# shuwang127/SRCNN_Cpp

Measured on AMD Instinct MI355X. Metric: SRCNN Y-channel Mpixels/sec, higher is better.
Workload: dtype f32; 1 GPU; 1 x 3840x2160 luma plane per GPU per step (1920x1080 x2.0, BASELINE configs[1]), fused conv path, mfma arithmetic, inputs resident in HBM; frames_per_gpu=1, width=3840, height=2160, mode=mfma, seam_deferral=True, output_checksum=584152

## Files before the change

### srcnn_cpp_amd/csrc/srcnn_kernels.h

```cpp
#pragma once
#include <hip/hip_runtime.h>
#include <stddef.h>
#include <stdint.h>

namespace srcnn {

constexpr int FW = 128;
constexpr int YP = FW + 8;
constexpr int YR = 16;
constexpr int NWAVES = FW / 32;
constexpr int NTHREADS = NWAVES * 64;

enum StripMode { MODE_FUSED = 0, MODE_L12 = 1, MODE_L3 = 2 };

constexpr int NFRAG_L1 = 82;
constexpr int NFRAG_L2 = 32;
constexpr int NFRAG_L3 = 16;
constexpr int NFRAG_B2 = 16;
constexpr int NFRAG_L2U = 32;
constexpr int NFRAG_B2U = 16;
constexpr int NFRAG_L3U = 16;
constexpr int FRAG_L2 = NFRAG_L1, FRAG_L3 = FRAG_L2 + NFRAG_L2, FRAG_B2 = FRAG_L3 + NFRAG_L3,
              FRAG_L2U = FRAG_B2 + NFRAG_B2, FRAG_B2U = FRAG_L2U + NFRAG_L2U, FRAG_L3U = FRAG_B2U + NFRAG_B2U;
constexpr int NFRAG = FRAG_L3U + NFRAG_L3U;

__host__ __device__ constexpr int acc_row(int r, int h) { return (r & 3) + 8 * (r >> 2) + 4 * h; }
__host__ __device__ constexpr int row_chan(int i) { return 2 * ((i & 3) + 4 * (i >> 3)) + ((i >> 2) & 1); }

__host__ __device__ constexpr int l3_row_tap(int i)
{
    const int r = (i & 3) + 4 * (i >> 3), h = (i >> 2) & 1, s = r / 5, m = r % 5, n = h ? 3 + s : s;
    return (r < 15 && n < 5) ? 5 * m + n : -1;
}
__host__ __device__ constexpr bool l3_row_is_scale(int i)
{
    const int r = (i & 3) + 4 * (i >> 3), h = (i >> 2) & 1;
    return h == 1 && r >= 10 && r < 15;
}

constexpr int S16_FRAG_L2 = 24, S16_FRAG_L3 = 32, S16_NFRAG = 36;
constexpr size_t S16_TABLE_BYTES = (size_t)S16_NFRAG * 64 * 16 + 2 * 16 * sizeof(float);
__host__ __device__ constexpr int l1s_tap(int b, int h, int e)
{
    const int n = 4 * b + e / 2, u = e & 1;
    if (n < 20) return (2 * (n % 5) + u < 9) ? 9 * (n / 5 + 5 * h) + 2 * (n % 5) + u : -1;
    if (n < 23) {
        const int jj = 4 * h + 2 * (n - 20) + u;
        return (h == 0 ? jj <= 3 : (jj >= 4 && jj <= 8)) ? 36 + jj : -1;
    }
    return (u == 0 && h == 0) ? 81 : -1;
}

struct StripParams {
    const uint8_t *src;
    long src_stride, src_frame_pitch;
    int src_row0;
    const uint8_t *src_top, *src_bot;
    long halo_stride;
    int src_row1;
    const float *planes_in;
    float *planes_out;
    long pl_stride, pl_pitch, pl_frame_pitch;
    uint8_t *dst;
    float *pre;
    long dst_stride, dst_frame_pitch;
    int dst_row0;
    const float *wfrag;
    const uint32_t *wfrag16;
    float *sink;
    float b3;
    int width, height;
    int row_begin, row_end;
    int seg_rows, n_strips, n_segs;
    const int *items;
    int items_per_frame;
    int seams_per_frame;
    float *seam;
    float *cseam;
    int strips_total;
    int tune;
    uint8_t *flag;
    float fix_delta, fix_scale;
    float fix_kl, fix_abs;
    unsigned *fix_counters;
};

enum { FIX_N_SCAT = 0, FIX_N_DENSE = 1, FIX_N_CHANGED = 2, FIX_MAX_DEV = 3, FIX_N_RERUN = 4,
       FIX_MAX_RATIO = 5,
       FIX_TOTALS = 6,
       FIX_WORD_STRIDE = 64,
       FIX_NEXT_ITEM = 6,
       FIX_NEXT_RERUN = 7,
       FIX_REGIONS = 8, FIX_REGION0 = 8 * FIX_WORD_STRIDE,
       FIX_COUNTERS = FIX_REGION0 + FIX_REGIONS * FIX_WORD_STRIDE };
struct FixParams {
    const uint8_t *src;
    long src_stride;
    int src_row0;
    const uint8_t *src_top, *src_bot;
    long halo_stride;
    int src_row1;
    uint8_t *dst;
    const uint8_t *flag;
    long dst_stride;
    int dst_row0;
    int width, height, row_begin, row_end;
    const float *wraw;
// ... 172 lines not shown
```

### srcnn_cpp_amd/csrc/srcnn_mfma.hip

```cpp
#include "srcnn_kernels.h"

#include <type_traits>

#ifndef SRCNN_SAFE_HAZARDS
#define SRCNN_SAFE_HAZARDS 0
#endif
#if SRCNN_SAFE_HAZARDS
#define SRCNN_KNS safe
#else
#define SRCNN_KNS fast
#endif

namespace srcnn {
namespace SRCNN_KNS {

typedef float f32x16 __attribute__((ext_vector_type(16)));
typedef float f32x2 __attribute__((ext_vector_type(2)));

#define MFMA(a, b, c) __builtin_amdgcn_mfma_f32_32x32x2f32((a), (b), (c), 0, 0, 0)

__device__ __forceinline__ f32x16 mfma_first(float a, float b, const f32x16 &c)
{
#if SRCNN_SAFE_HAZARDS
    return MFMA(a, b, c);
#endif
    f32x16 d;
    asm volatile("v_mfma_f32_32x32x2_f32 %0, %1, %2, %3" : "=&v"(d) : "v"(a), "v"(b), "v"(c));
    return d;
}
__device__ __forceinline__ f32x16 mfma_first0(float a, float b)
{
#if SRCNN_SAFE_HAZARDS
    const f32x16 z = {0};
    return MFMA(a, b, z);
#endif
    f32x16 d;
    asm volatile("v_mfma_f32_32x32x2_f32 %0, %1, %2, 0" : "=&v"(d) : "v"(a), "v"(b));
    return d;
}


__device__ __forceinline__ int clampi(int v, int lo, int hi) { return min(max(v, lo), hi); }

__device__ __forceinline__ unsigned lane_off(unsigned x)
{
    asm volatile("" : "+v"(x));
    return x;
}
template <typename T>
__device__ __forceinline__ __attribute__((address_space(1))) T *scalar_base(T *p)
{
    __attribute__((address_space(1))) T *g = (__attribute__((address_space(1))) T *)p;
    asm volatile("" : "+s"(g));
    return g;
}

template <typename T>
__device__ __forceinline__ T *uniform_ptr(T *p)
{
    const unsigned long long a = (unsigned long long)p;
    const unsigned lo = __builtin_amdgcn_readfirstlane((unsigned)a), hi = __builtin_amdgcn_readfirstlane((unsigned)(a >> 32));
    return (T *)(((unsigned long long)hi << 32) | lo);
}

__device__ __forceinline__ void lds_barrier()
{
    asm volatile("s_waitcnt lgkmcnt(0)\n\ts_barrier" ::: "memory");
}

__device__ __forceinline__ float relu(float x)
{
    float r;
    asm("v_max_f32 %0, 0, %1" : "=v"(r) : "v"(x));
    return r;
}

__device__ const signed char CSEAM_TERMS[15][9] = {
    {4, 0, 124, 1, 125, 2, 126, 3, 127}, {3, 0, 125, 1, 126, 2, 127, 0, 0}, {1, 0, 126, 0, 0, 0, 0, 0, 0},
    {1, 0, 127, 0, 0, 0, 0, 0, 0},       {1, 1, 127, 0, 0, 0, 0, 0, 0},     {1, 2, 0, 0, 0, 0, 0, 0, 0},
    {1, 3, 1, 0, 0, 0, 0, 0, 0},         {1, 4, 2, 0, 0, 0, 0, 0, 0},       {1, 1, 0, 0, 0, 0, 0, 0, 0},
    {1, 2, 1, 0, 0, 0, 0, 0, 0},         {1, 3, 2, 0, 0, 0, 0, 0, 0},       {1, 4, 3, 0, 0, 0, 0, 0, 0},
    {1, 3, 0, 0, 0, 0, 0, 0, 0},         {1, 4, 0, 0, 0, 0, 0, 0, 0},       {1, 4, 1, 0, 0, 0, 0, 0, 0}};

struct CseamLane {
    int cnt, off[4];
};
__device__ __forceinline__ CseamLane cseam_lane(int e)
{
    CseamLane cl = {0, {0, 0, 0, 0}};
    if (e < 15) {
        const signed char *t = CSEAM_TERMS[e];
        cl.cnt = t[0];
#pragma unroll
        for (int i = 0; i < 4; ++i) cl.off[i] = i < t[0] ? t[1 + 2 * i] * FW + t[2 + 2 * i] : 0;
    }
    return cl;
}
__device__ __forceinline__ void cseam_export(const float *tile, float *dst, int e, const CseamLane &cl)
{
    const float a = tile[cl.off[0]], b = tile[cl.off[1]], c = tile[cl.off[2]], d = tile[cl.off[3]];
    float v = a;
    v = cl.cnt > 1 ? v + b : v;
    v = cl.cnt > 2 ? v + c : v;
    v = cl.cnt > 3 ? v + d : v;
    if (cl.cnt > 0) dst[(unsigned)e] = v;
}

__device__ __forceinline__ void relu_pairs(f32x16 &a, const f32x2 ones)
{
#if SRCNN_SAFE_HAZARDS
#pragma unroll
    for (int q = 0; q < 16; ++q) a[q] = __builtin_fmaxf(a[q], 0.f);
    return;
#endif
#pragma unroll
    for (int q = 0; q < 8; ++q) {
        f32x2 pr = {a[2 * q], a[2 * q + 1]};
        asm("v_pk_mul_f32 %0, %0, %1 clamp" : "+v"(pr) : "s"(ones));
        a[2 * q] = pr.x;
        a[2 * q + 1] = pr.y;
    }
}

constexpr bool fast_kernel(int mode, bool pre, int diag)
{
    (void)diag;
    return mode == MODE_FUSED && !pre;
}

template <int MODE, bool PRE, int DIAG = 0, bool FIX = false, bool HALO3 = false>
__device__ __forceinline__ void strip_body(const StripParams &p)
{
    static_assert(!FIX || (MODE == MODE_FUSED && !PRE && DIAG == 0), "flags belong to the production fused kernel");
    static_assert(!HALO3 || (MODE == MODE_FUSED && !PRE && DIAG == 0), "halo buffers belong to the production fused kernel");
    if constexpr (FIX) {
        if (blockIdx.x == 0)
            for (int i = threadIdx.x; i < FIX_COUNTERS; i += 256) p.fix_counters[i] = 0u;
    }
    unsigned long long lt[4] = {0, 0, 0, 0};
    if constexpr (DIAG == 2) lt[0] = __builtin_amdgcn_s_memrealtime();
    extern __shared__ __attribute__((aligned(16))) char smem[];
    float *ylds = reinterpret_cast<float *>(smem);
    float *fbuf = (MODE == MODE_L3) ? ylds : ylds + 2 * YR * YP;

    const int tid = threadIdx.x;
    const int lane = tid & 63;
    const int wave = __builtin_amdgcn_readfirstlane(tid >> 6);
    const int j = lane & 31;
    const int half = lane >> 5;

    constexpr int HALO = (MODE == MODE_L12) ? 0 : 2;

    const int W = p.width, H = p.height;
    int bid = blockIdx.x;
    int strip, frame = 0, ys, ye, seam_up = -1, seam_dn = -1;
    if (p.items) {
        frame = bid / p.items_per_frame;
        const int *it = p.items + ITEM_INTS * (bid - frame * p.items_per_frame);
        strip = it[0];
        ys = it[1];
        ye = it[2];
        if constexpr (MODE == MODE_FUSED) {
            seam_up = it[3] >= 0 ? it[3] + frame * p.seams_per_frame : -1;
            seam_dn = it[4] >= 0 ? it[4] + frame * p.seams_per_frame : -1;
        }
        if (ys >= ye) return;
    } else {
        if (!(p.tune & 8)) {
            const int nwg = gridDim.x, q = nwg >> 3, r = nwg & 7, xcd = bid & 7;
            bid = (xcd < r ? xcd * (q + 1) : r * (q + 1) + (xcd - r) * q) + (bid >> 3);
        }
        strip = bid % p.n_strips;
        bid /= p.n_strips;
        const int seg = bid % p.n_segs;
        frame = bid / p.n_segs;
        ys = p.row_begin + seg * p.seg_rows;
        ye = min(ys + p.seg_rows, p.row_end);
    }

    const bool cs = (MODE != MODE_L12) && p.cseam != nullptr;
    const CseamLane cl = cseam_lane((cs && threadIdx.x < 64 && (threadIdx.x & 31) < 15 &&
                                     (threadIdx.x < 32 || fast_kernel(MODE, PRE, DIAG)))
                                        ? (int)(threadIdx.x & 31) : 15);
    const int halo_c = cs ? 0 : HALO;
    const int xs = strip * (FW - 2 * halo_c);
    const int gx0 = xs - halo_c;
    float *cs_row0 = (cs && wave == 0)
                         ? p.cseam + (((long)frame * p.strips_total + strip) * (p.row_end - p.row_begin) - p.row_begin) * CSEAM_FLOATS
                         : nullptr;
    const bool top_open = seam_up >= 0, bot_open = seam_dn >= 0;
    const int f_lo = top_open ? ys : max(ys - HALO, 0);
    const int f_hi = bot_open ? ye : min(ye + HALO, H);
    const int out_lo = top_open ? ys + 2 : ys, out_hi = bot_open ? ye - 2 : ye;

    const float *wf = p.wfrag + lane;
    float w1f[2][41], w2f[32], w3f[16];
    f32x16 b2v = {0};
    if constexpr (MODE != MODE_L3) {
#pragma unroll
        for (int t = 0; t < 2; ++t)
#pragma unroll
            for (int s = 0; s < 41; ++s) w1f[t][s] = wf[(t * 41 + s) * 64];
        constexpr int L2 = (MODE == MODE_L12) ? FRAG_L2U : FRAG_L2, B2 = (MODE == MODE_L12) ? FRAG_B2U : FRAG_B2;
#pragma unroll
        for (int q = 0; q < 32; ++q) w2f[q] = wf[(L2 + q) * 64];
#pragma unroll
        for (int q = 0; q < 16; ++q) b2v[q] = wf[(B2 + q) * 64];
    }
    if constexpr (MODE != MODE_L12) {
        constexpr int L3 = (MODE == MODE_L3) ? FRAG_L3U : FRAG_L3;
#pragma unroll
        for (int q = 0; q < 16; ++q) w3f[q] = wf[(L3 + q) * 64];
    }
    const f32x2 ones = {1.0f, 1.0f};

    const uint8_t *srcf = nullptr;
    int ycol = 0;
    if constexpr (MODE != MODE_L3) {
        srcf = p.src + (long)frame * p.src_frame_pitch;
        ycol = clampi(gx0 - 4 + tid, 0, W - 1);
    }
    const int y_last = min(H - 1, f_hi + 3);
    auto y_row = [&](int r) -> const uint8_t * {
        if constexpr (HALO3) {
            if (r < p.src_row0) return p.src_top + (long)(r - (p.src_row0 - 6)) * p.halo_stride;
            if (r >= p.src_row1) return p.src_bot + (long)(r - p.src_row1) * p.halo_stride;
        }
        return srcf + (long)(r - p.src_row0) * p.src_stride;
    };
    auto load_y = [&](int r) -> uint8_t {
        const uint8_t *row = y_row(clampi(r, 0, y_last));
        return row[(unsigned)ycol];
    };
    auto stage_y = [&](int r, uint8_t v) {
        const int slot = r & (YR - 1);
        const float fv = (float)v;
        ylds[slot * YP + tid] = fv;
        ylds[(slot + YR) * YP + tid] = fv;
    };
    if constexpr (MODE != MODE_L3) {
        if (tid < YP) {
            uint8_t v[9];
#pragma unroll
            for (int q = 0; q < 9; ++q) v[q] = load_y(f_lo - 4 + q);
#pragma unroll
            for (int q = 0; q < 9; ++q) stage_y(f_lo - 4 + q, v[q]);
        }
        __syncthreads();
    }
    asm volatile("s_waitcnt vmcnt(0)" ::: "memory");
    if constexpr (MODE != MODE_L3) {
#pragma unroll
        for (int t = 0; t < 2; ++t)
#pragma unroll
            for (int k = 0; k < 41; ++k) asm volatile("" : "+v"(w1f[t][k]));
#pragma unroll
        for (int q = 0; q < 32; ++q) asm volatile("" : "+v"(w2f[q]));
        asm volatile("" : "+v"(b2v));
    }
    if constexpr (MODE != MODE_L12) {
#pragma unroll
        for (int q = 0; q < 16; ++q) asm volatile("" : "+v"(w3f[q]));
    }

    if constexpr (DIAG == 2) lt[1] = __builtin_amdgcn_s_memrealtime();

    const int xi = 32 * wave + j;
    const int gx = gx0 + xi;


    constexpr bool FASTK = fast_kernel(MODE, PRE, DIAG);
    static_assert(!FIX || FASTK, "the flag threshold reads plane 5 through the FAST kernels' column offsets");
    constexpr int FSLOT = 6 * FW;
    int xn[5] = {0, 0, 0, 0, 0};
    bool px_ok = false;
    if constexpr (MODE != MODE_L12) {
#pragma unroll
        for (int n = 0; n < 5; ++n) {
            xn[n] = clampi(clampi(gx + n - 2, 0, W - 1) - gx0, 0, FW - 1);
            if constexpr (FASTK) xn[n] += n * FW + half * FSLOT;
        }
        px_ok = cs ? (gx < W) && (xi >= 2 || strip == 0) && (xi < FW - 2 || strip == p.strips_total - 1)
                   : (xi >= HALO) && (xi < FW - HALO) && (gx < W);
    }
    CseamLane cl2 = cl;
    if constexpr (FASTK) {
#pragma unroll
        for (int i = 0; i < 4; ++i) cl2.off[i] += half * FSLOT;
    }
    float R[4][3] = {{0.f, 0.f, 0.f}, {0.f, 0.f, 0.f}, {0.f, 0.f, 0.f}, {0.f, 0.f, 0.f}};
    long o_out = (long)frame * p.dst_frame_pitch + (long)(f_lo - 3 - p.dst_row0) * p.dst_stride;
    long o_src = (long)(min(f_lo + 5, y_last) - p.src_row0) * p.src_stride;
    long o_pl = (long)frame * p.pl_frame_pitch + (long)(MODE == MODE_L3 ? min(f_lo + 1, H - 1) : f_lo) * p.pl_stride;
    auto scale_thr = [&](const float *fr) -> float {
        float s1 = fr[xn[0] + 5 * FW];
#pragma unroll
        for (int n = 1; n < 5; ++n) s1 += fr[xn[n] + (5 - n) * FW];
        return fix_threshold(s1, p.fix_delta, p.fix_kl, p.fix_abs);
    };
    auto finalize = [&](long o, float acc, bool ok, const float *fr) {
        const float v = acc + p.b3;
        auto row = scalar_base(p.dst + o);
        if (ok) row[lane_off((unsigned)gx)] = (uint8_t)clampi((int)v, 0, 255);
        if constexpr (FIX) {
            auto frow = scalar_base(p.flag + o);
            const float thr = scale_thr(fr);
            if (ok) frow[lane_off((unsigned)gx)] = fix_code(v, thr, p.fix_delta, p.fix_scale);
        }
        if constexpr (PRE) {
            float *prow = p.pre + o;
            if (ok) prow[(unsigned)gx] = v;
        }
    };
    auto ftile = [&](int g, int slot) -> float * {
        if constexpr (FASTK) return fbuf + ((4 - ((g + slot) & 3)) & 3) * FSLOT;
        else return fbuf + (((g & 1) * 3 + slot) * 6) * FW;
    };
    auto vertical = [&](int f, const f32x16 &t) {
        const int fplane = 3 * half * FW + xi;
        if (top_open && f < ys + SEAM_ROWS) {
            const int r = f - ys;
            float *o = p.seam + ((long)seam_up * SEAM_FLOATS + seam_t_off(r)) * NTHREADS + tid;
#pragma unroll
            for (int s = 0; s < 3; ++s)
#pragma unroll
                for (int m = 1; m < 5; ++m)
                    if (m > r) o[(s * (4 - r) + (m - r - 1)) * NTHREADS] = t[5 * s + m];
        }
        if (f > 0) {
            float *fo = ftile(f, 0) + fplane;
#pragma unroll
            for (int s = 0; s < 3; ++s) {
                fo[s * FW] = R[3][s] + t[5 * s + 4];
                R[3][s] = R[2][s] + t[5 * s + 3];
                R[2][s] = R[1][s] + t[5 * s + 2];
                R[1][s] = R[0][s] + t[5 * s + 1];
                R[0][s] = t[5 * s];
            }
// ... 20 lines not shown
        const float *fr = ftile(g, slot);
#pragma unroll
        for (int n = 0; n < 5; ++n) hv[n] = FASTK ? fr[xn[n]] : fr[n * FW + xn[n]];
    };
    auto hp_use = [&](int g, int slot) {
        float acc = hv[0];
#pragma unroll
        for (int n = 1; n < 5; ++n) acc += hv[n];
        const int y = g - 2 + slot;
        const bool rows_ok = (y >= out_lo) && (y < out_hi) && (!FASTK || half == 0);
        finalize(slot == 0 ? o_out : o_out + (long)slot * p.dst_stride, acc, px_ok && rows_ok, ftile(g, slot));
        if (cs_row0 && rows_ok) cseam_export(ftile(g, slot), cs_row0 + y * CSEAM_FLOATS, lane, FASTK ? cl2 : cl);
    };
    const unsigned st2 = (unsigned)gx + (half ? 0u : (unsigned)p.dst_stride);
    const unsigned cs2 = (unsigned)(lane & 31) + (half ? 0u : (unsigned)CSEAM_FLOATS);
    const int do_cs = __builtin_amdgcn_readfirstlane((cs && wave == 0) ? 1 : 0);
    auto hp2_load = [&](int slot) {
        const float *fr = fbuf + slot * FSLOT;
#pragma unroll
        for (int n = 0; n < 5; ++n) hv[n] = fr[xn[n]];
    };
    float v2 = 0.f;
    auto hp2_use = [&](int f, int slot) {
        float acc = hv[0];
#pragma unroll
        for (int n = 1; n < 5; ++n) acc += hv[n];
        const float v = acc + p.b3;
        auto row = scalar_base(p.dst + (o_out - p.dst_stride));
        if (px_ok) row[lane_off(st2)] = (uint8_t)clampi((int)v, 0, 255);
        if constexpr (FIX) {
            v2 = v;
            const float *fr = fbuf + slot * FSLOT;
#pragma unroll
            for (int n = 0; n < 5; ++n) hv[n] = fr[xn[n] + (5 - n) * FW];
        }
        if (do_cs) {
            const float *tile = fbuf + slot * FSLOT;
            const float a = tile[cl2.off[0]], b = tile[cl2.off[1]], c = tile[cl2.off[2]], d = tile[cl2.off[3]];
            float e = a;
            e = cl2.cnt > 1 ? e + b : e;
            e = cl2.cnt > 2 ? e + c : e;
            e = cl2.cnt > 3 ? e + d : e;
            auto dst = scalar_base(cs_row0 + (f - 4) * CSEAM_FLOATS);
            if (cl2.cnt > 0) dst[cs2] = e;
        }
    };

    auto hp2_flag = [&]() {
        float s1 = hv[0];
#pragma unroll
        for (int n = 1; n < 5; ++n) s1 += hv[n];
        const float thr = fix_threshold(s1, p.fix_delta, p.fix_kl, p.fix_abs);
        auto frow = scalar_base(p.flag + (o_out - p.dst_stride));
        if (px_ok) frow[lane_off(st2)] = fix_code(v2, thr, p.fix_delta, p.fix_scale);
    };

    f32x16 d2n = {0};
    const unsigned pl_lane = (MODE == MODE_L12) ? (unsigned)(half * p.pl_pitch + gx)
                                                : (unsigned)(half * p.pl_pitch + clampi(gx, 0, W - 1));
    auto load_planes_at = [&](long o) {
        const float *q = p.planes_in + o;
        const unsigned lo = lane_off(pl_lane * 4u);
#pragma unroll
        for (int r = 0; r < 16; ++r)
            d2n[r] = __builtin_nontemporal_load((const __attribute__((address_space(1))) float *)((const __attribute__((address_space(1))) char *)scalar_base(q + (long)(2 * r) * p.pl_pitch) + lo));
    };
    if constexpr (MODE == MODE_L3) load_planes_at((long)frame * p.pl_frame_pitch + (long)f_lo * p.pl_stride);
    auto drain = [&](int g) {
        const int nslots = (g == H - 1) ? 3 : 1;
        for (int slot = 0; slot < nslots; ++slot) {
            hp_load(g, slot);
            hp_use(g, slot);
        }
    };
    auto row = [&](int f, auto ph_tag) {
        constexpr int PH = decltype(ph_tag)::value;
        constexpr bool FAST = PH >= 0;
        const int g = f - 1;
        const bool hp = FAST ? (PH & 1) != 0 : (MODE != MODE_L12) && (g >= f_lo);
        constexpr int SLOT_W = (4 - PH) & 3;
        constexpr int SLOT_R = (4 - ((PH + 3) & 3)) & 3;

        f32x16 d2;
        if constexpr (MODE != MODE_L3) {
            unsigned ynext;
            asm volatile("" : "=v"(ynext));
            if constexpr (HALO3) {
                const uint8_t *yr = uniform_ptr(y_row(min(f + 5, y_last)));
                if (tid < YP) ynext = scalar_base(yr)[lane_off((unsigned)ycol)];
            } else {
                if (tid < YP) ynext = scalar_base(srcf + o_src)[lane_off((unsigned)ycol)];
                if (f + 5 < y_last) o_src += p.src_stride;
            }

            const float *yb = ylds + ((f - 4) & (YR - 1)) * YP + xi;
            const float *ybN = yb + half;
            const float *ybW = yb + (half ? YP - 8 : 0);
            auto ldb = [&](int s) -> float {
                const int ki = (2 * s) / 9, kj = (2 * s) % 9;
                if (s == 40) return half ? 1.0f : yb[8 * YP + 8];
                if (kj == 8) return ybW[ki * YP + kj];
                return ybN[ki * YP + kj];
            };
            f32x16 a0 = {0}, a1 = {0};
            auto layer1 = [&](auto with_pb) {
                constexpr bool PB = decltype(with_pb)::value;
                constexpr int PF = 3;
                float bq[41];
#pragma unroll
                for (int s = 0; s < PF; ++s) bq[s] = ldb(s);
#pragma unroll
                for (int s = 0; s < 41; ++s) {
                    if (s + PF < 41) bq[s + PF] = ldb(s + PF);
                    if constexpr (PB && MODE != MODE_L12) {
                        if constexpr (FAST) {
                            if (s == 2) hp2_load(SLOT_R);
                            if (s == 8) hp2_use(f, SLOT_R);
                            if constexpr (FIX) {
                                if (s == 14) hp2_flag();
                            }
                        } else {
                            if (s == 2) hp_load(g, 0);
                            if (s == 8) hp_use(g, 0);
                        }
                    }
                    a0 = MFMA(w1f[0][s], bq[s], a0);
                    a1 = MFMA(w1f[1][s], bq[s], a1);
                    __builtin_amdgcn_sched_barrier(0);
                }
            };
            if constexpr (FAST) {
                layer1(std::integral_constant<bool, (PH & 1) != 0>{});
            } else {
                if (hp) layer1(std::true_type{});
                else layer1(std::false_type{});
            }
            relu_pairs(a0, ones);
            relu_pairs(a1, ones);
            __builtin_amdgcn_sched_barrier(0);

            d2 = mfma_first(w2f[0], a0[0], b2v);
#pragma unroll
            for (int r = 1; r < 16; ++r) d2 = MFMA(w2f[r], a0[r], d2);
#pragma unroll
            for (int r = 0; r < 16; ++r) d2 = MFMA(w2f[16 + r], a1[r], d2);
            __builtin_amdgcn_sched_barrier(0);
            if constexpr (MODE == MODE_L12) {
#pragma unroll
                for (int r = 0; r < 16; ++r) d2[r] = relu(d2[r]);
            } else {
                relu_pairs(d2, ones);
            }
            __builtin_amdgcn_sched_barrier(0);

            asm volatile("" : "+v"(ynext));
            if (tid < YP) stage_y(f + 5, (uint8_t)ynext);

            if constexpr (MODE == MODE_L12) {
                if (gx < W) {
                    float *o = p.planes_out + o_pl;
                    const unsigned lo = lane_off(pl_lane * 4u);
#pragma unroll
                    for (int r = 0; r < 16; ++r)
                        __builtin_nontemporal_store(d2[r], (__attribute__((address_space(1))) float *)((__attribute__((address_space(1))) char *)scalar_base(o + (long)(2 * r) * p.pl_pitch) + lo));
                }
            }
        } else {
            d2 = d2n;
            load_planes_at(o_pl);
            if constexpr (FAST) {
                if constexpr ((PH & 1) != 0) {
                    hp2_load(SLOT_R);
                    hp2_use(f, SLOT_R);
                }
            } else if (hp) {
                hp_load(g, 0);
                hp_use(g, 0);
            }
        }

        if constexpr (MODE != MODE_L12) {
            f32x16 t = {0};
            if constexpr (MODE == MODE_FUSED) {
                t = mfma_first0(w3f[0], d2[0]);
#pragma unroll
                for (int r = 1; r < 16; ++r) t = MFMA(w3f[r], d2[r], t);
            } else {
#pragma unroll
                for (int r = 0; r < 16; ++r) t = MFMA(w3f[r], d2[r], t);
            }
            __builtin_amdgcn_sched_barrier(0);
            if constexpr (FAST) {
                float *fo = fbuf + SLOT_W * FSLOT + 3 * half * FW + xi;
#pragma unroll
                for (int s = 0; s < 3; ++s) {
                    fo[s * FW] = R[3][s] + t[5 * s + 4];
#ifndef SRCNN_ABL_NO_CHAIN_ADDS
                    R[3][s] = R[2][s] + t[5 * s + 3];
                    R[2][s] = R[1][s] + t[5 * s + 2];
                    R[1][s] = R[0][s] + t[5 * s + 1];
                    R[0][s] = t[5 * s];
#endif
                    asm volatile("" : "+v"(R[0][s]), "+v"(R[1][s]), "+v"(R[2][s]), "+v"(R[3][s]));
                }
            } else {
                vertical(f, t);
            }
        }

        if constexpr (FASTK) __builtin_amdgcn_sched_barrier(0);
        lds_barrier();
        if constexpr (FASTK) __builtin_amdgcn_sched_barrier(0);
        o_out += p.dst_stride;
        if constexpr (MODE == MODE_L3) {
            if (f + 1 < H - 1) o_pl += p.pl_stride;
        } else {
            o_pl += p.pl_stride;
        }
    };
    {
        int f = f_lo;
        if constexpr (FASTK) {
            const int f_a = (f_lo + 6 + 1) & ~1;
            const int f_b = min(f_hi, H - 1) & ~1;
            for (; f < f_hi && f < f_a; ++f) row(f, std::integral_constant<int, -1>{});
            if ((f & 2) && f + 2 <= f_b) {
                row(f, std::integral_constant<int, 2>{});
                row(f + 1, std::integral_constant<int, 3>{});
                f += 2;
            }
            for (; f + 4 <= f_b; f += 4) {
                row(f, std::integral_constant<int, 0>{});
                row(f + 1, std::integral_constant<int, 1>{});
                row(f + 2, std::integral_constant<int, 2>{});
                row(f + 3, std::integral_constant<int, 3>{});
            }
            if (f + 2 <= f_b) {
                row(f, std::integral_constant<int, 0>{});
                row(f + 1, std::integral_constant<int, 1>{});
                f += 2;
            }
        }
        for (; f < f_hi; ++f) row(f, std::integral_constant<int, -1>{});
    }
    if constexpr (MODE != MODE_L12) {
        if (f_hi > f_lo) drain(f_hi - 1);
    }
    if constexpr (DIAG == 2) lt[2] = __builtin_amdgcn_s_memrealtime();
    if (bot_open) {
        float *o = p.seam + (long)seam_dn * SEAM_FLOATS * NTHREADS + tid;
#pragma unroll
        for (int k = 0; k < 4; ++k)
#pragma unroll
            for (int s = 0; s < 3; ++s) o[(k * 3 + s) * NTHREADS] = R[k][s];
    }
    if constexpr (DIAG == 2) {
        asm volatile("s_waitcnt vmcnt(0)" ::: "memory");
        lt[3] = __builtin_amdgcn_s_memrealtime();
        if (lane == 0) {
            unsigned long long *o = reinterpret_cast<unsigned long long *>(p.sink + 256) + ((long)blockIdx.x * NWAVES + wave) * 8;
            o[0] = lt[0];
            o[1] = lt[1];
            o[2] = lt[2];
            o[3] = lt[3];
            o[4] = (unsigned long long)(f_hi - f_lo);
            o[5] = (unsigned long long)__builtin_amdgcn_s_getreg((31 << 11) | (0 << 6) | 4) |
                   ((unsigned long long)__builtin_amdgcn_s_getreg((31 << 11) | (0 << 6) | 20) << 32);
// ... 267 lines not shown
```

### srcnn_cpp_amd/csrc/srcnn_model.cpp

```cpp
#include "srcnn_ctx.h"

using namespace srcnn;
using namespace srcnn::host;

namespace srcnn {
namespace host {

int scale_exponent(double bound)
{
    if (!(bound > 0.0) || !std::isfinite(bound)) return 0;
    int e = 0;
    (void)std::frexp(bound * (1.0 + 1.0 / 65536.0), &e);
    return e;
}

float fixup_delta(const float *w1, const float *b1, const float *w2, const float *b2, const float *w3, double margin)
{
    double a1[64], m2 = 0.0, s3 = 0.0;
    for (int c = 0; c < 64; ++c) {
        double s = 0.0;
        for (int t = 0; t < 81; ++t) s += std::max(w1[c * 81 + t], 0.f);
        a1[c] = std::max(0.0, 255.0 * s + b1[c]);
    }
    for (int k = 0; k < 32; ++k) {
        double s = b2[k];
        for (int i = 0; i < 64; ++i) s += (double)std::max(w2[k * 64 + i], 0.f) * a1[i];
        m2 = std::max(m2, s);
    }
    for (int i = 0; i < 800; ++i) s3 += (double)w3[i] * w3[i];
    const double d = margin * std::ldexp(1.0, -24) * std::sqrt(s3) * m2 + 4.0 * std::ldexp(1.0, -24) * 256.0;
    if (!std::isfinite(d)) return 0.25f;
    return (float)std::min(0.25, std::max(d, 1e-6));
}

void layer_scales(const float *w1, const float *b1, const float *w2, const float *b2, int *e1, int *e2)
{
    double a1[64], m1 = 0.0, m2 = 0.0;
    for (int c = 0; c < 64; ++c) {
        double s = 0.0;
        for (int t = 0; t < 81; ++t) s += std::max(w1[c * 81 + t], 0.f);
        a1[c] = std::max(0.0, 255.0 * s + b1[c]);
        m1 = std::max(m1, a1[c]);
    }
    for (int k = 0; k < 32; ++k) {
        double s = b2[k];
        for (int i = 0; i < 64; ++i) s += (double)std::max(w2[k * 64 + i], 0.f) * a1[i];
        m2 = std::max(m2, s);
    }
    *e1 = scale_exponent(m1);
    *e2 = scale_exponent(m2);
}

void pack_fragments(const float *w1 , const float *b1, const float *w2 ,
                    const float *b2, const float *w3 , float *out )
{
    int e1, e2;
    layer_scales(w1, b1, w2, b2, &e1, &e2);
    for (int l = 0; l < 64; ++l) {
        const int i = l & 31, kk = l >> 5;
        const int ch = row_chan(i);
        for (int t = 0; t < 2; ++t)
            for (int s = 0; s < 41; ++s) {
                const int tap = 2 * s + kk, c = 32 * t + ch;
                out[(t * 41 + s) * 64 + l] = std::ldexp(tap < 81 ? w1[c * 81 + tap] : b1[c], -e1);
            }
        for (int t = 0; t < 2; ++t)
            for (int r = 0; r < 16; ++r) {
                const float w = w2[ch * 64 + 32 * t + 2 * r + kk];
                out[(FRAG_L2 + t * 16 + r) * 64 + l] = std::ldexp(w, e1 - e2);
                out[(FRAG_L2U + t * 16 + r) * 64 + l] = std::ldexp(w, e1);
            }
        for (int r = 0; r < 16; ++r) {
            const int tap = l3_row_tap(i);
            const float w = tap >= 0 ? w3[(2 * r + kk) * 25 + tap] : 0.f;
            float a = 0.f;
            if (l3_row_is_scale(i))
                for (int t = 0; t < 25; ++t) a = std::max(a, std::fabs(w3[(2 * r + kk) * 25 + t]));
            out[(FRAG_L3 + r) * 64 + l] = std::ldexp(tap >= 0 ? w : a, e2);
            out[(FRAG_L3U + r) * 64 + l] = w;
        }
        for (int r = 0; r < 16; ++r) {
            out[(FRAG_B2 + r) * 64 + l] = std::ldexp(b2[2 * r + kk], -e2);
            out[(FRAG_B2U + r) * 64 + l] = b2[2 * r + kk];
        }
    }
}

void split16(float w, float scale, uint16_t *hi, uint16_t *lo)
{
    const float ws = w * scale;
    const _Float16 h = (_Float16)ws;
    const _Float16 l = (_Float16)(ws - (float)h);
    std::memcpy(hi, &h, 2);
    std::memcpy(lo, &l, 2);
}

void pack_fragments16(const float *w1 , const float *b1, const float *w2 ,
                      const float *b2, const float *w3 , uint8_t *out )
{
    constexpr float SCALE = 16384.f, SCALE1 = 2048.f;
    uint16_t *tab = reinterpret_cast<uint16_t *>(out);
    auto slot = [&](int frag, int l, int e) -> uint16_t * { return tab + ((size_t)frag * 64 + l) * 8 + e; };
    for (int l = 0; l < 64; ++l) {
        const int m = l & 31, h = l >> 5;
        for (int e = 0; e < 8; ++e) {
            for (int t = 0; t < 2; ++t)
                for (int b = 0; b < 6; ++b) {
                    const int tap = l1s_tap(b, h, e), c = 32 * t + m;
                    const float w = tap < 0 ? 0.f : (tap == 81 ? b1[c] : w1[c * 81 + tap]);
                    split16(w, tap == 81 ? 0.125f : SCALE1, slot((2 * t) * 6 + b, l, e), slot((2 * t + 1) * 6 + b, l, e));
                }
            for (int b = 0; b < 4; ++b) {
                const int c1 = 32 * (b >> 1) + acc_row(8 * (b & 1) + e, h);
                split16(w2[m * 64 + c1], SCALE, slot(S16_FRAG_L2 + b, l, e), slot(S16_FRAG_L2 + 4 + b, l, e));
            }
            for (int b = 0; b < 2; ++b) {
                const int c2 = acc_row(8 * b + e, h), tap = l3_row_tap(m);
                float a = 0.f;
                if (l3_row_is_scale(m))
                    for (int t = 0; t < 25; ++t) a = std::max(a, std::fabs(w3[c2 * 25 + t]));
                split16(tap >= 0 ? w3[c2 * 25 + tap] : a, SCALE, slot(S16_FRAG_L3 + b, l, e),
                        slot(S16_FRAG_L3 + 2 + b, l, e));
            }
        }
    }
    float *b2t = reinterpret_cast<float *>(out + (size_t)S16_NFRAG * 64 * 16);
    for (int h = 0; h < 2; ++h)
        for (int r = 0; r < 16; ++r) b2t[h * 16 + r] = b2[acc_row(r, h)] * 0.0625f;
}

bool split16_range_ok(const float *w1, const float *b1, const float *w2, const float *b2, const float *w3)
{
    float a1[64], wmax1 = 0.f, wmax23 = 0.f, a1max = 0.f, a2max = 0.f;
    for (int c = 0; c < 64; ++c) {
        double s = 0;
        for (int t = 0; t < 81; ++t) {
            s += std::max(w1[c * 81 + t], 0.f);
            wmax1 = std::max(wmax1, std::fabs(w1[c * 81 + t]));
        }
        a1[c] = std::max(0.f, (float)(255.0 * s + b1[c]));
        a1max = std::max(a1max, a1[c]);
        wmax1 = std::max(wmax1, std::fabs(b1[c]) / 256.f);
    }
    for (int k = 0; k < 32; ++k) {
        double s = b2[k];
        for (int i = 0; i < 64; ++i) {
            s += (double)std::max(w2[k * 64 + i], 0.f) * a1[i];
            wmax23 = std::max(wmax23, std::fabs(w2[k * 64 + i]));
// ... 157 lines not shown
```

### srcnn_cpp_amd/csrc/srcnn_probe.hip

```cpp
#include "srcnn_kernels.h"

#include <vector>

namespace srcnn {

typedef float f32x16 __attribute__((ext_vector_type(16)));
typedef float f32x2 __attribute__((ext_vector_type(2)));
#define PROBE_WAIT() do { if constexpr (WAIT) asm volatile("s_nop 15\n\ts_nop 15" ::: "memory"); } while (0)

template <bool WAIT>
__global__ __launch_bounds__(256) void interlock_probe_kernel(const float *__restrict__ in, float *__restrict__ out, int iters)
{
    const int t = blockIdx.x * blockDim.x + threadIdx.x;
    float a = in[t], b = in[t + 4096], w = in[t + 2048] * 0.25f, r = 0.f;
    const f32x2 ones = {1.0f, 1.0f};
    f32x16 cinit;
    for (int q = 0; q < 16; ++q) cinit[q] = in[(t + 64 * q) & 4095] * 0.125f;
    for (int k = 0; k < iters; ++k) {
        f32x16 acc, acc2, acc3;
        asm volatile("v_mfma_f32_32x32x2_f32 %0, %1, %2, 0" : "=&v"(acc) : "v"(a), "v"(b));
        PROBE_WAIT();
#pragma unroll
        for (int q = 0; q < 8; ++q) {
            f32x2 pr = {acc[2 * q], acc[2 * q + 1]};
            asm volatile("v_pk_mul_f32 %0, %0, %1 clamp" : "+v"(pr) : "s"(ones));
            acc[2 * q] = pr.x;
            acc[2 * q + 1] = pr.y;
        }
        PROBE_WAIT();
        asm volatile("v_mfma_f32_32x32x2_f32 %0, %1, %2, %3" : "=&v"(acc2) : "v"(w), "v"(acc[0]), "v"(cinit));
        PROBE_WAIT();
#pragma unroll
        for (int q = 1; q < 16; ++q) acc2 = __builtin_amdgcn_mfma_f32_32x32x2f32(w, acc[q], acc2, 0, 0, 0);
        PROBE_WAIT();
#pragma unroll
        for (int q = 0; q < 8; ++q) {
            f32x2 pr = {acc2[2 * q], acc2[2 * q + 1]};
            asm volatile("v_pk_mul_f32 %0, %0, %1 clamp" : "+v"(pr) : "s"(ones));
            acc2[2 * q] = pr.x;
            acc2[2 * q + 1] = pr.y;
        }
        PROBE_WAIT();
        asm volatile("v_mfma_f32_32x32x2_f32 %0, %1, %2, 0" : "=&v"(acc3) : "v"(w), "v"(acc2[0]));
        PROBE_WAIT();
#pragma unroll
        for (int q = 1; q < 16; ++q) acc3 = __builtin_amdgcn_mfma_f32_32x32x2f32(w, acc2[q], acc3, 0, 0, 0);
        float s = 0.f;
#pragma unroll
        for (int q = 0; q < 16; ++q) s += acc3[q] + acc2[q] * 0.5f + acc[q] * 0.25f;
        r = r * 0.5f + s;
        a = a * 0.5f + 0.25f * w;
        b = b * 0.75f + 0.1f;
    }
    out[t] = r;
}

long interlock_probe_mismatches(int device, hipStream_t st)
{
    constexpr int kThreads = 256, kBlocks = 512, n = kThreads * kBlocks;
    int prev = -1;
    if (hipGetDevice(&prev) != hipSuccess) prev = -1;
    if (hipSetDevice(device) != hipSuccess) return -1;
    std::vector<float> h((size_t)n + 4096);
    for (size_t i = 0; i < h.size(); ++i) h[i] = (float)((i * 2654435761u) % 1000) / 250.f - 2.f;
    float *d_in = nullptr, *d_a = nullptr, *d_b = nullptr;
    long bad = -1;
    if (hipMalloc(&d_in, h.size() * 4) == hipSuccess && hipMalloc(&d_a, (size_t)n * 4) == hipSuccess &&
        hipMalloc(&d_b, (size_t)n * 4) == hipSuccess &&
        hipMemcpyAsync(d_in, h.data(), h.size() * 4, hipMemcpyHostToDevice, st) == hipSuccess) {
        bad = 0;
        std::vector<float> ra((size_t)n), rb((size_t)n);
        for (int rep = 0; rep < 2 && bad >= 0; ++rep) {
            hipLaunchKernelGGL(interlock_probe_kernel<false>, dim3(kBlocks), dim3(kThreads), 0, st, d_in, d_a, 24);
            hipLaunchKernelGGL(interlock_probe_kernel<true>, dim3(kBlocks), dim3(kThreads), 0, st, d_in, d_b, 24);
            if (hipGetLastError() != hipSuccess || hipMemcpyAsync(ra.data(), d_a, (size_t)n * 4, hipMemcpyDeviceToHost, st) != hipSuccess ||
                hipMemcpyAsync(rb.data(), d_b, (size_t)n * 4, hipMemcpyDeviceToHost, st) != hipSuccess ||
                hipStreamSynchronize(st) != hipSuccess) {
                bad = -1;
                break;
            }
            long nonzero = 0;
            for (int i = 0; i < n; ++i) {
                bad += ra[(size_t)i] != rb[(size_t)i];
                nonzero += rb[(size_t)i] != 0.f;
            }
            if (nonzero < n / 2) bad += n;
        }
    }
    (void)hipStreamSynchronize(st);
    if (d_in) (void)hipFree(d_in);
    if (d_a) (void)hipFree(d_a);
    if (d_b) (void)hipFree(d_b);
    if (prev >= 0 && prev != device) (void)hipSetDevice(prev);
    return bad;
}

}
```

Measured before the change: 8759 MPix/s.

## Replace layer-1 bias MFMA tap with a 32x32x1 tap plus packed bias-add ReLU

Layer 1 previously folded the last weight tap and the bias into one extra 32x32x2 MFMA step, using a constant 1.0 input on one half to supply the bias. Now the 81st tap runs as a single 32x32x1 MFMA that updates both accumulators at once. The bias is loaded from an LDS table and applied together with ReLU through a packed add-with-clamp, which replaces the old multiply-by-one clamp. The weight fragment layout is reordered to match, and layer 3 reuses a dead accumulator as its output register to save registers. The trade-off is extra LDS loads and careful scheduling against MFMA hazards, so a probe kernel is added to check the interlock.

```diff
diff --git a/srcnn_cpp_amd/csrc/srcnn_kernels.h b/srcnn_cpp_amd/csrc/srcnn_kernels.h
--- a/srcnn_cpp_amd/csrc/srcnn_kernels.h
+++ b/srcnn_cpp_amd/csrc/srcnn_kernels.h
@@ -13,16 +13,18 @@
 
 enum StripMode { MODE_FUSED = 0, MODE_L12 = 1, MODE_L3 = 2 };
 
-constexpr int NFRAG_L1 = 82;
+constexpr int NFRAG_L1 = 81;
 constexpr int NFRAG_L2 = 32;
 constexpr int NFRAG_L3 = 16;
 constexpr int NFRAG_B2 = 16;
 constexpr int NFRAG_L2U = 32;
 constexpr int NFRAG_B2U = 16;
 constexpr int NFRAG_L3U = 16;
+constexpr int NFRAG_B1 = 1;
 constexpr int FRAG_L2 = NFRAG_L1, FRAG_L3 = FRAG_L2 + NFRAG_L2, FRAG_B2 = FRAG_L3 + NFRAG_L3,
               FRAG_L2U = FRAG_B2 + NFRAG_B2, FRAG_B2U = FRAG_L2U + NFRAG_L2U, FRAG_L3U = FRAG_B2U + NFRAG_B2U;
-constexpr int NFRAG = FRAG_L3U + NFRAG_L3U;
+constexpr int FRAG_B1 = FRAG_L3U + NFRAG_L3U;
+constexpr int NFRAG = FRAG_B1 + NFRAG_B1;
 
 __host__ __device__ constexpr int acc_row(int r, int h) { return (r & 3) + 8 * (r >> 2) + 4 * h; }
 __host__ __device__ constexpr int row_chan(int i) { return 2 * ((i & 3) + 4 * (i >> 3)) + ((i >> 2) & 1); }
diff --git a/srcnn_cpp_amd/csrc/srcnn_mfma.hip b/srcnn_cpp_amd/csrc/srcnn_mfma.hip
--- a/srcnn_cpp_amd/csrc/srcnn_mfma.hip
+++ b/srcnn_cpp_amd/csrc/srcnn_mfma.hip
@@ -16,6 +16,8 @@
 
 typedef float f32x16 __attribute__((ext_vector_type(16)));
 typedef float f32x2 __attribute__((ext_vector_type(2)));
+typedef float f32x4 __attribute__((ext_vector_type(4)));
+typedef float f32x32 __attribute__((ext_vector_type(32)));
 
 #define MFMA(a, b, c) __builtin_amdgcn_mfma_f32_32x32x2f32((a), (b), (c), 0, 0, 0)
 
@@ -37,6 +39,14 @@
     f32x16 d;
     asm volatile("v_mfma_f32_32x32x2_f32 %0, %1, %2, 0" : "=&v"(d) : "v"(a), "v"(b));
     return d;
+}
+__device__ __forceinline__ f32x16 mfma_first0_over(float a, float b, f32x16 &dead)
+{
+#if SRCNN_SAFE_HAZARDS
+    return mfma_first0(a, b);
+#endif
+    asm volatile("v_mfma_f32_32x32x2_f32 %0, %1, %2, 0" : "+v"(dead) : "v"(a), "v"(b));
+    return dead;
 }
 
 
@@ -122,6 +132,49 @@
     }
 }
 
+__device__ __forceinline__ void mfma_tap_2b(float w, float y, f32x16 &a0, f32x16 &a1, [[maybe_unused]] int half)
+{
+#if SRCNN_SAFE_HAZARDS
+    a0 = MFMA(w, half ? 0.f : y, a0);
+    a1 = MFMA(w, half ? y : 0.f, a1);
+    return;
+#endif
+    f32x32 c = __builtin_shufflevector(a0, a1, 0, 1, 2, 3, 4, 5, 6, 7, 8, 9, 10, 11, 12, 13, 14, 15, 16, 17, 18, 19, 20, 21, 22, 23,
+                                       24, 25, 26, 27, 28, 29, 30, 31);
+    c = __builtin_amdgcn_mfma_f32_32x32x1f32(w, y, c, 0, 0, 0);
+    a0 = __builtin_shufflevector(c, c, 0, 1, 2, 3, 4, 5, 6, 7, 8, 9, 10, 11, 12, 13, 14, 15);
+    a1 = __builtin_shufflevector(c, c, 16, 17, 18, 19, 20, 21, 22, 23, 24, 25, 26, 27, 28, 29, 30, 31);
+}
+
+template <int H>
+__device__ __forceinline__ void bias_relu_pairs(f32x16 &a, const f32x4 &b0, const f32x4 &b1)
+{
+#pragma unroll
+    for (int q = 0; q < 4; ++q) {
+        const f32x4 &b = q < 2 ? b0 : b1;
+        f32x2 pr = {a[8 * H + 2 * q], a[8 * H + 2 * q + 1]};
+        const f32x2 bp = {b[2 * (q & 1)], b[2 * (q & 1) + 1]};
+        asm("v_pk_add_f32 %0, %0, %1 clamp" : "+v"(pr) : "v"(bp));
+        a[8 * H + 2 * q] = pr.x;
+        a[8 * H + 2 * q + 1] = pr.y;
+    }
+}
+
+__device__ __forceinline__ void bias_relu_safe(f32x16 &a, const f32x4 *bt)
+{
+    f32x4 cur = bt[0];
+#pragma unroll
+    for (int k = 0; k < 4; ++k) {
+        f32x4 nxt = cur;
+        if (k < 3) nxt = bt[k + 1];
+        __builtin_amdgcn_sched_barrier(0);
+#pragma unroll
+        for (int q = 0; q < 4; ++q) a[4 * k + q] = __builtin_fmaxf(a[4 * k + q] + cur[q], 0.f);
+        __builtin_amdgcn_sched_barrier(0);
+        cur = nxt;
+    }
+}
+
 constexpr bool fast_kernel(int mode, bool pre, int diag)
 {
     (void)diag;
@@ -142,6 +195,7 @@
     extern __shared__ __attribute__((aligned(16))) char smem[];
     float *ylds = reinterpret_cast<float *>(smem);
     float *fbuf = (MODE == MODE_L3) ? ylds : ylds + 2 * YR * YP;
+    __shared__ __attribute__((aligned(16))) float btab[MODE == MODE_L3 ? 4 : 64];
 
     const int tid = threadIdx.x;
     const int lane = tid & 63;
@@ -194,13 +248,14 @@
     const int out_lo = top_open ? ys + 2 : ys, out_hi = bot_open ? ye - 2 : ye;
 
     const float *wf = p.wfrag + lane;
-    float w1f[2][41], w2f[32], w3f[16];
+    float w1f[2][40], w1t = 0.f, w2f[32], w3f[16];
     f32x16 b2v = {0};
     if constexpr (MODE != MODE_L3) {
 #pragma unroll
         for (int t = 0; t < 2; ++t)
 #pragma unroll
-            for (int s = 0; s < 41; ++s) w1f[t][s] = wf[(t * 41 + s) * 64];
+            for (int s = 0; s < 40; ++s) w1f[t][s] = wf[(t * 40 + s) * 64];
+        w1t = wf[80 * 64];
         constexpr int L2 = (MODE == MODE_L12) ? FRAG_L2U : FRAG_L2, B2 = (MODE == MODE_L12) ? FRAG_B2U : FRAG_B2;
 #pragma unroll
         for (int q = 0; q < 32; ++q) w2f[q] = wf[(L2 + q) * 64];
@@ -239,6 +294,7 @@
         ylds[(slot + YR) * YP + tid] = fv;
     };
     if constexpr (MODE != MODE_L3) {
+        if (tid < 64) btab[tid] = p.wfrag[FRAG_B1 * 64 + tid];
         if (tid < YP) {
             uint8_t v[9];
 #pragma unroll
@@ -253,7 +309,8 @@
 #pragma unroll
         for (int t = 0; t < 2; ++t)
 #pragma unroll
-            for (int k = 0; k < 41; ++k) asm volatile("" : "+v"(w1f[t][k]));
+            for (int k = 0; k < 40; ++k) asm volatile("" : "+v"(w1f[t][k]));
+        asm volatile("" : "+v"(w1t));
 #pragma unroll
         for (int q = 0; q < 32; ++q) asm volatile("" : "+v"(w2f[q]));
         asm volatile("" : "+v"(b2v));
@@ -440,6 +497,7 @@
         constexpr int SLOT_R = (4 - ((PH + 3) & 3)) & 3;
 
         f32x16 d2;
+        f32x16 a0 = {0}, a1 = {0};
         if constexpr (MODE != MODE_L3) {
             unsigned ynext;
             asm volatile("" : "=v"(ynext));
@@ -456,20 +514,28 @@
             const float *ybW = yb + (half ? YP - 8 : 0);
             auto ldb = [&](int s) -> float {
                 const int ki = (2 * s) / 9, kj = (2 * s) % 9;
-                if (s == 40) return half ? 1.0f : yb[8 * YP + 8];
+                if (s == 40) return yb[8 * YP + 8];
                 if (kj == 8) return ybW[ki * YP + kj];
                 return ybN[ki * YP + kj];
             };
-            f32x16 a0 = {0}, a1 = {0};
+            const f32x4 *bt = reinterpret_cast<const f32x4 *>(btab + 32 * half);
+            [[maybe_unused]] f32x4 b1v[4];
             auto layer1 = [&](auto with_pb) {
                 constexpr bool PB = decltype(with_pb)::value;
                 constexpr int PF = 3;
+                [[maybe_unused]] constexpr int PB1 = 34;
                 float bq[41];
 #pragma unroll
                 for (int s = 0; s < PF; ++s) bq[s] = ldb(s);
 #pragma unroll
-                for (int s = 0; s < 41; ++s) {
+                for (int s = 0; s < 40; ++s) {
                     if (s + PF < 41) bq[s + PF] = ldb(s + PF);
+#if !SRCNN_SAFE_HAZARDS
+                    if (s == PB1) {
+#pragma unroll
+                        for (int q = 0; q < 4; ++q) b1v[q] = bt[q];
+                    }
+#endif
                     if constexpr (PB && MODE != MODE_L12) {
                         if constexpr (FAST) {
                             if (s == 2) hp2_load(SLOT_R);
@@ -486,6 +552,8 @@
                     a1 = MFMA(w1f[1][s], bq[s], a1);
                     __builtin_amdgcn_sched_barrier(0);
                 }
+                mfma_tap_2b(w1t, bq[40], a0, a1, half);
+                __builtin_amdgcn_sched_barrier(0);
             };
             if constexpr (FAST) {
                 layer1(std::integral_constant<bool, (PH & 1) != 0>{});
@@ -493,8 +561,21 @@
                 if (hp) layer1(std::true_type{});
                 else layer1(std::false_type{});
             }
-            relu_pairs(a0, ones);
-            relu_pairs(a1, ones);
+#if SRCNN_SAFE_HAZARDS
+            bias_relu_safe(a0, bt);
+            bias_relu_safe(a1, bt + 4);
+#else
+            bias_relu_pairs<0>(a0, b1v[0], b1v[1]);
+            __builtin_amdgcn_sched_barrier(0);
+            const f32x4 c0 = bt[4], c1 = bt[5];
+            __builtin_amdgcn_sched_barrier(0);
+            bias_relu_pairs<1>(a0, b1v[2], b1v[3]);
+            __builtin_amdgcn_sched_barrier(0);
+            const f32x4 c2 = bt[6], c3 = bt[7];
+            __builtin_amdgcn_sched_barrier(0);
+            bias_relu_pairs<0>(a1, c0, c1);
+            bias_relu_pairs<1>(a1, c2, c3);
+#endif
             __builtin_amdgcn_sched_barrier(0);
 
             d2 = mfma_first(w2f[0], a0[0], b2v);
@@ -540,7 +621,7 @@
         if constexpr (MODE != MODE_L12) {
             f32x16 t = {0};
             if constexpr (MODE == MODE_FUSED) {
-                t = mfma_first0(w3f[0], d2[0]);
+                t = mfma_first0_over(w3f[0], d2[0], a0);
 #pragma unroll
                 for (int r = 1; r < 16; ++r) t = MFMA(w3f[r], d2[r], t);
             } else {
diff --git a/srcnn_cpp_amd/csrc/srcnn_model.cpp b/srcnn_cpp_amd/csrc/srcnn_model.cpp
--- a/srcnn_cpp_amd/csrc/srcnn_model.cpp
+++ b/srcnn_cpp_amd/csrc/srcnn_model.cpp
@@ -60,10 +60,12 @@
         const int i = l & 31, kk = l >> 5;
         const int ch = row_chan(i);
         for (int t = 0; t < 2; ++t)
-            for (int s = 0; s < 41; ++s) {
-                const int tap = 2 * s + kk, c = 32 * t + ch;
-                out[(t * 41 + s) * 64 + l] = std::ldexp(tap < 81 ? w1[c * 81 + tap] : b1[c], -e1);
-            }
+            for (int s = 0; s < 40; ++s) out[(t * 40 + s) * 64 + l] = std::ldexp(w1[(32 * t + ch) * 81 + 2 * s + kk], -e1);
+        out[80 * 64 + l] = std::ldexp(w1[(32 * kk + ch) * 81 + 80], -e1);
+        {
+            const int h = l >> 5, t = (l >> 4) & 1, r = l & 15;
+            out[FRAG_B1 * 64 + l] = std::ldexp(b1[32 * t + 2 * r + h], -e1);
+        }
         for (int t = 0; t < 2; ++t)
             for (int r = 0; r < 16; ++r) {
                 const float w = w2[ch * 64 + 32 * t + 2 * r + kk];
diff --git a/srcnn_cpp_amd/csrc/srcnn_probe.hip b/srcnn_cpp_amd/csrc/srcnn_probe.hip
--- a/srcnn_cpp_amd/csrc/srcnn_probe.hip
+++ b/srcnn_cpp_amd/csrc/srcnn_probe.hip
@@ -55,6 +55,50 @@
     out[t] = r;
 }
 
+template <bool WAIT>
+__global__ __launch_bounds__(256) void l1_bias_probe_kernel(const float *__restrict__ in, float *__restrict__ out, int iters)
+{
+    typedef float f32x32 __attribute__((ext_vector_type(32)));
+    const int t = blockIdx.x * blockDim.x + threadIdx.x;
+    float a = in[t], b = in[t + 4096], w = in[t + 2048] * 0.25f, r = 0.f;
+    f32x16 cinit;
+    f32x2 bias[16];
+    for (int q = 0; q < 16; ++q) {
+        cinit[q] = in[(t + 64 * q) & 4095] * 0.125f;
+        bias[q] = f32x2{in[(t + 7 + 32 * q) & 4095], in[(t + 19 + 32 * q) & 4095]} * 0.25f;
+    }
+    for (int k = 0; k < iters; ++k) {
+        const f32x16 z = {0};
+        f32x16 a0 = __builtin_amdgcn_mfma_f32_32x32x2f32(a, b, z, 0, 0, 0);
+        f32x16 a1 = __builtin_amdgcn_mfma_f32_32x32x2f32(w, b, z, 0, 0, 0);
+        f32x32 c = __builtin_shufflevector(a0, a1, 0, 1, 2, 3, 4, 5, 6, 7, 8, 9, 10, 11, 12, 13, 14, 15, 16, 17, 18, 19, 20, 21, 22,
+                                           23, 24, 25, 26, 27, 28, 29, 30, 31);
+        c = __builtin_amdgcn_mfma_f32_32x32x1f32(w, a, c, 0, 0, 0);
+        __builtin_amdgcn_sched_barrier(0);
+        PROBE_WAIT();
+#pragma unroll
+        for (int q = 0; q < 16; ++q) {
+            f32x2 pr = {c[2 * q], c[2 * q + 1]};
+            asm volatile("v_pk_add_f32 %0, %0, %1 clamp" : "+v"(pr) : "v"(bias[q]));
+            c[2 * q] = pr.x;
+            c[2 * q + 1] = pr.y;
+        }
+        PROBE_WAIT();
+        f32x16 acc2;
+        asm volatile("v_mfma_f32_32x32x2_f32 %0, %1, %2, %3" : "=&v"(acc2) : "v"(w), "v"(c[0]), "v"(cinit));
+        PROBE_WAIT();
+#pragma unroll
+        for (int q = 1; q < 32; ++q) acc2 = __builtin_amdgcn_mfma_f32_32x32x2f32(w, c[q], acc2, 0, 0, 0);
+        float s = 0.f;
+#pragma unroll
+        for (int q = 0; q < 16; ++q) s += acc2[q] + c[q] * 0.5f + c[16 + q] * 0.25f;
+        r = r * 0.5f + s;
+        a = a * 0.5f + 0.25f * w;
+        b = b * 0.75f + 0.1f;
+    }
+    out[t] = r;
+}
+
 long interlock_probe_mismatches(int device, hipStream_t st)
 {
     constexpr int kThreads = 256, kBlocks = 512, n = kThreads * kBlocks;
@@ -70,9 +114,14 @@
         hipMemcpyAsync(d_in, h.data(), h.size() * 4, hipMemcpyHostToDevice, st) == hipSuccess) {
         bad = 0;
         std::vector<float> ra((size_t)n), rb((size_t)n);
-        for (int rep = 0; rep < 2 && bad >= 0; ++rep) {
-            hipLaunchKernelGGL(interlock_probe_kernel<false>, dim3(kBlocks), dim3(kThreads), 0, st, d_in, d_a, 24);
-            hipLaunchKernelGGL(interlock_probe_kernel<true>, dim3(kBlocks), dim3(kThreads), 0, st, d_in, d_b, 24);
+        for (int rep = 0; rep < 4 && bad >= 0; ++rep) {
+            if (rep < 2) {
+                hipLaunchKernelGGL(interlock_probe_kernel<false>, dim3(kBlocks), dim3(kThreads), 0, st, d_in, d_a, 24);
+                hipLaunchKernelGGL(interlock_probe_kernel<true>, dim3(kBlocks), dim3(kThreads), 0, st, d_in, d_b, 24);
+            } else {
+                hipLaunchKernelGGL(l1_bias_probe_kernel<false>, dim3(kBlocks), dim3(kThreads), 0, st, d_in, d_a, 24);
+                hipLaunchKernelGGL(l1_bias_probe_kernel<true>, dim3(kBlocks), dim3(kThreads), 0, st, d_in, d_b, 24);
+            }
             if (hipGetLastError() != hipSuccess || hipMemcpyAsync(ra.data(), d_a, (size_t)n * 4, hipMemcpyDeviceToHost, st) != hipSuccess ||
                 hipMemcpyAsync(rb.data(), d_b, (size_t)n * 4, hipMemcpyDeviceToHost, st) != hipSuccess ||
                 hipStreamSynchronize(st) != hipSuccess) {
```

Measured after the change: 8824 MPix/s, median of 6. Within noise of the previous version (+0.7%).
